# marco-conciatori-public/weed_instance_segmentation

Hardware: AMD Instinct MI355X
Metric: images/sec at 1024x1024 bs=8 per GPU (Mask2Former R50, 100 queries, fp32 forward-only) (higher is better)
Workload: dtype f32

## Files before the change

include/wm2f.h:

```cpp
#ifndef WM2F_H
#define WM2F_H

#include <stdint.h>

#ifdef __cplusplus
extern "C" {
#endif

#define WM2F_VERSION 100

#define WM2F_F32 0
#define WM2F_BF16 1
#define WM2F_I32 2
#define WM2F_U8 3
#define WM2F_U16 4
#define WM2F_I64 5

#define WM2F_OK 0
#define WM2F_EINVAL (-1)
#define WM2F_EUNSUPPORTED (-2)
#define WM2F_ELAUNCH (-3)

#define WM2F_MAX_LEVELS 8

// ... 181 lines not shown
                             int N, int Hi, int Wi, int stride, int relu, int config, int pieces, void* stream);
int wm2f_conv1x1_split_gn_fwd_p(const void* x, const void* w_split, const void* bias, void* out, void* stats_out, int G_out,
                                const void* norm_stats, const void* norm_gamma, const void* norm_beta, int norm_G, float norm_eps,
                                int norm_relu, int B, int K, int N, int Hi, int Wi, int stride, int config, int pieces,
                                void* stream);
int wm2f_conv1x1_split_dual_fwd_p(const void* x1, const void* ws1, const void* x2, const void* ws2, const void* bias, void* out,
                                  int B, int K1, int K2, int N, int Ho, int Wo, int H2, int W2, int stride2, int config,
                                  int pieces, void* stream);
int wm2f_conv3x3_split_fwd_p(const void* x, const void* w_split, const void* bias, void* out, int B, int Cin, int N, int Hi,
                             int Wi, int stride, int relu, int config, int pieces, void* stream);
int wm2f_conv3x3_split_stats_fwd_p(const void* x, const void* w_split, void* out, void* stats_out, int G_out, int B, int Cin,
                                   int N, int Hi, int Wi, int stride, int config, int pieces, void* stream);
int wm2f_stem7x7_pool_fwd_p(const void* x, const void* w_split, const void* bias, void* out, int B, int Cin, int N, int Hi,
                            int Wi, int grid, int pieces, void* stream);

int wm2f_swin_linear_split_fwd_p(const void* x, const void* w_split, const void* bias, const void* residual, void* out0,
                                 void* out1, void* out2, int64_t M, int K, int N, int epilogue, int n_out, int config,
                                 int pieces, void* stream);
int wm2f_swin_linear_split_config(int64_t M, int N, int pieces, int n_cu);
int wm2f_swin_linear_split_configs(void);

int64_t wm2f_token_wgrad_workspace(int64_t M, int N, int K);
int wm2f_token_wgrad_bf16(const void* dy, const void* x, void* dw, void* db, void* workspace, int64_t M, int N, int K,
                          void* stream);
int wm2f_token_wgrad_f32(const void* dy, const void* x, void* dw, void* db, void* workspace, int64_t M, int N, int K,
                         void* stream);
int wm2f_tokens_to_nchw(const void* tokens, void* out, int B, int S, int C, int start, int HW, void* stream);
int wm2f_group_norm_tokens(const void* x, const void* bias, const void* gamma, const void* beta, void* tokens,
                           void* stats_ws, int B, int C, int G, int HW, int S, int start, float eps, void* stream);
int wm2f_resize_bilinear(const void* x, void* y, int NC, int H, int W, int Ho, int Wo, void* stream);
// ... 261 lines not shown
```

weed_instance_segmentation_amd/_lib.py:

```python
from __future__ import annotations

import ctypes
import os
from ctypes import POINTER, c_char_p, c_float, c_int, c_int32, c_int64, c_void_p

HERE = os.path.dirname(os.path.abspath(__file__))
LIB_PATH = os.path.join(HERE, "libwm2f.so")
PROF_LIB_PATH = os.path.join(HERE, "libwm2f_prof.so")
if os.environ.get("WM2F_PROF_LIB"):
    PROF_LIB_PATH = os.environ["WM2F_PROF_LIB"]

WM2F_F32 = 0
WM2F_BF16 = 1
WM2F_I32 = 2
WM2F_U8 = 3
WM2F_U16 = 4
WM2F_I64 = 5
WM2F_CCL_VALUE, WM2F_CCL_BINARY, WM2F_CCL_RGB = 0, 1, 2
WM2F_CCL_MAX_COLORS = 16
WM2F_POLY_MAX_SIDE = 16384
WM2F_POLY_MAX_COORD = 1 << 24
WM2F_RLE_MAX_IDS = 1024
WM2F_AUG_MAX_VIRTUAL = 65536
WM2F_TILE_MAX_SIDE, WM2F_TILE_MAX_IDS, WM2F_TILE_MAX_TILES, WM2F_TILE_MAX_PAIRS = 16384, 256, 1024, 16384
# ... 85 lines not shown
    "wm2f_conv3x3_split_config": (c_int, [_I, _I, _I, _I]),
    "wm2f_conv3x3_split_fwd": (c_int, [_P, _P, _P, _P, _I, _I, _I, _I, _I, _I, _I, _I, _P]),
    "wm2f_conv1x1_split_gn_fwd": (c_int, [_P, _P, _P, _P, _P, _I, _P, _P, _P, _I, c_float, _I, _I, _I, _I, _I, _I, _I, _I, _P]),
    "wm2f_conv3x3_split_stats_fwd": (c_int, [_P, _P, _P, _P, _I, _I, _I, _I, _I, _I, _I, _I, _P]),
    "wm2f_group_norm_act_apply": (c_int, [_P, _P, _P, _P, _P, _P, _I, _I, _I, _I, _I, _I, _I, c_float, _I, _P]),
    "wm2f_group_norm_tokens_apply": (c_int, [_P, _P, _P, _P, _P, _P, _I, _I, _I, _I, _I, _I, c_float, _P]),
    "wm2f_stem7x7_pool_fwd":(c_int, [_P, _P, _P, _P, _I, _I, _I, _I, _I, _I, _P]),
    "wm2f_token_linear_split_fwd_p": (c_int, [_P, _P, _P, _P, _P, _P, _P, _P, _P, c_int64, _I, _I, _I, c_int64, c_float, _I, _I, _P]),
    "wm2f_token_ffn_split_fwd_p": (c_int, [_P, _P, _P, _P, _P, _P, _P, _P, _P, _P, _P, c_int64, _I, _I, _I, c_int64, c_float, _I, _P]),
    "wm2f_conv1x1_split_fwd_p": (c_int, [_P, _P, _P, _P, _P, _I, _I, _I, _I, _I, _I, _I, _I, _I, _P]),
    "wm2f_conv1x1_split_gn_fwd_p": (c_int, [_P, _P, _P, _P, _P, _I, _P, _P, _P, _I, c_float, _I, _I, _I, _I, _I, _I, _I, _I, _I, _P]),
    "wm2f_conv1x1_split_dual_fwd_p": (c_int, [_P, _P, _P, _P, _P, _P, _I, _I, _I, _I, _I, _I, _I, _I, _I, _I, _I, _P]),
    "wm2f_conv3x3_split_fwd_p": (c_int, [_P, _P, _P, _P, _I, _I, _I, _I, _I, _I, _I, _I, _I, _P]),
    "wm2f_conv3x3_split_stats_fwd_p": (c_int, [_P, _P, _P, _P, _I, _I, _I, _I, _I, _I, _I, _I, _I, _P]),
    "wm2f_stem7x7_pool_fwd_p": (c_int, [_P, _P, _P, _P, _I, _I, _I, _I, _I, _I, _I, _P]),
    "wm2f_swin_linear_split_fwd_p": (c_int, [_P, _P, _P, _P, _P, _P, _P, c_int64, _I, _I, _I, _I, _I, _I, _P]),
    "wm2f_swin_linear_split_config": (c_int, [c_int64, _I, _I, _I]),
    "wm2f_swin_linear_split_configs": (c_int, []),
    "wm2f_token_wgrad_workspace": (c_int64, [c_int64, _I, _I]),
    "wm2f_token_wgrad_bf16": (c_int, [_P, _P, _P, _P, _P, c_int64, _I, _I, _P]),
    "wm2f_token_wgrad_f32": (c_int, [_P, _P, _P, _P, _P, c_int64, _I, _I, _P]),
    "wm2f_tokens_to_nchw": (c_int, [_P, _P, _I, _I, _I, _I, _I, _P]),
    "wm2f_group_norm_tokens": (c_int, [_P, _P, _P, _P, _P, _P, _I, _I, _I, _I, _I, _I, c_float, _P]),
    "wm2f_resize_bilinear": (c_int, [_P, _P, _I, _I, _I, _I, _I, _P]),
    "wm2f_resize_pyramid": (c_int, [_P, _P, _P, _P, _I, _I, _I, _P]),
    "wm2f_bias_relu_maxpool": (c_int, [_P, _P, _P, _I, _I, _I, _I, _P]),
    "wm2f_group_norm_act": (c_int, [_P, _P, _P, _P, _P, _P, _I, _I, _I, _I, _I, _I, _I, c_float, _I, _P]),
    "wm2f_point_sample_fwd": (c_int, [_P, _I, _P, _P, _P, _I, _I, _I, _I, _P]),
    "wm2f_point_sample_bwd": (c_int, [_P, _P, _P, _P, _I, _I, _I, _I, _P]),
    "wm2f_labelmap_pair_counts": (c_int, [_P, _I, _P, _I, _P, _P, _P, _I, c_int64, _I, _I, _P]),
# ... 126 lines not shown
```

weed_instance_segmentation_amd/csrc/conv3x3_split.hip:

```cpp
#include "common.h"
#include "group_norm.h"

namespace wm2f {
namespace {

using f32x4 = __attribute__((ext_vector_type(4))) float;
using f32x8 = __attribute__((ext_vector_type(8))) float;
using bf16x8 = __attribute__((ext_vector_type(8))) __bf16;
typedef __attribute__((address_space(3))) void* lds_ptr_t;

constexpr int kWaves = 8;
constexpr int kThreads = kWaves * 64;
constexpr int kCT = 2;
constexpr int kKStep = 32;
constexpr int kFrag = 1024;
constexpr unsigned kOob = 0x80000000u;
constexpr float kBf16Max = 3.38953139e38f;

enum : int { kRaw = 0, kBias = 1, kBiasRelu = 2 };

__device__ __forceinline__ f32x8 widen(const bf16x8 v) {
  using u32x4 = __attribute__((ext_vector_type(4))) unsigned;
  const u32x4 w = __builtin_bit_cast(u32x4, v);
  f32x8 r;
// ... 21 lines not shown
    if constexpr (P >= 3) {
      const f32x8 r2 = r1 - widen(m);
      l = __builtin_convertvector(r2, bf16x8);
    }
  }
}

struct C3Args {
  const float *x, *bias;
  const void* ws;
  float* out;
  int Cin, N;
  int Hi, Wi, Wo, P, stride;
  double* stats;
  int G, cpg;
};

__device__ __forceinline__ void c3_barrier() {
  asm volatile("s_waitcnt vmcnt(0)" ::: "memory");
  __builtin_amdgcn_s_barrier();
  asm volatile("" ::: "memory");
}

template <int NRT, int WN, int EPI, bool STATS = false, int P = 3>
__global__ __launch_bounds__(kThreads) void conv3x3_split_kernel(C3Args a) {
  static_assert(P >= 1 && P <= 3, "one, two or three pieces");
  extern __shared__ __attribute__((aligned(16))) unsigned char smem[];
  constexpr int kRowTiles = WN * NRT;
  constexpr int kPanelBytes = kRowTiles * P * kFrag;
  constexpr int kPieces = kRowTiles * P;
  constexpr int kPT = (kWaves / WN) * kCT * 16;
  const int tid = threadIdx.x, lane = tid & 63, wave = __builtin_amdgcn_readfirstlane(tid >> 6);
  const int wn = wave % WN, wp = wave / WN;
  const int g = lane >> 4, j = lane & 15;
  const int nb = blockIdx.x, b = blockIdx.z;
  const int n_wg = nb * kRowTiles * 16;
  const int p_w = blockIdx.y * kPT + wp * kCT * 16;
  const int n_cb = a.Cin / kKStep;
  const int n_ks = 9 * n_cb;
  const int HWi = a.Hi * a.Wi;

// ... 20 lines not shown
    tap_ok[c] = m;
  }
  const unsigned ch_bytes = (unsigned)HWi * 4;

  f32x8 xr[kCT];
  auto issue = [&](int it) {
    const int cb = it / 9, tap = it - 9 * cb;
    const int dy = tap / 3, dx = tap - 3 * dy;
    unsigned char* dst = smem + (it & 1) * kPanelBytes;
    const int src = ((tap * n_cb + cb) * (a.N / 16) + n_wg / 16) * 3 * kFrag;
    for (int f = wave; f < kPieces; f += kWaves) {
      const int fs = P == 3 ? f : (f / P) * 3 + f % P;
      __builtin_amdgcn_raw_ptr_buffer_load_lds(w_rs, (lds_ptr_t)(dst + f * kFrag), 16, lane * 16, src + fs * kFrag, 0, 0);
    }
    const int kb = (cb * kKStep * HWi + dy * a.Wi + dx) * 4;
#pragma unroll
    for (int c = 0; c < kCT; ++c) {
      const unsigned o = (tap_ok[c] >> tap) & 1u ? (unsigned)(xo[c] + kb) : kOob;
#pragma unroll
      for (int i = 0; i < 8; ++i)
        xr[c][i] = __builtin_bit_cast(float, __builtin_amdgcn_raw_buffer_load_b32(x_rs, o, i * ch_bytes, 0));
    }
  };

  issue(0);
  c3_barrier();

  f32x4 acc[NRT][kCT];
#pragma unroll
  for (int rt = 0; rt < NRT; ++rt)
#pragma unroll
    for (int c = 0; c < kCT; ++c) acc[rt][c] = (f32x4){0.f, 0.f, 0.f, 0.f};

  for (int it = 0; it < n_ks; ++it) {
    bf16x8 bh[kCT], bm[kCT], bl[kCT];
#pragma unroll
    for (int c = 0; c < kCT; ++c) split3<P>(xr[c], bh[c], bm[c], bl[c]);
    if (it + 1 < n_ks) issue(it + 1);

    const unsigned char* panel = smem + (it & 1) * kPanelBytes + wn * NRT * P * kFrag;
    auto read_a = [&](bf16x8 (&dst)[3], int rt) {
#pragma unroll
      for (int p = 0; p < P; ++p) dst[p] = *reinterpret_cast<const bf16x8*>(panel + (rt * P + p) * kFrag + lane * 16);
    };
    auto six = [&](f32x4 acc_in, const bf16x8 (&av)[3], int cc) {
      f32x4 c = {0.f, 0.f, 0.f, 0.f};
      if constexpr (P == 3) {
        c = __builtin_amdgcn_mfma_f32_16x16x32_bf16(av[1], bm[cc], c, 0, 0, 0);
        c = __builtin_amdgcn_mfma_f32_16x16x32_bf16(av[2], bh[cc], c, 0, 0, 0);
        c = __builtin_amdgcn_mfma_f32_16x16x32_bf16(av[0], bl[cc], c, 0, 0, 0);
      }
      if constexpr (P >= 2) {
// ... 36 lines not shown
      for (int e = 0; e < 4; ++e) {
        float v = acc[rt][c][e];
        if (EPI != kRaw) v += bv[e];
        if (EPI == kBiasRelu) v = v < 0.f ? 0.f : v;
        __builtin_amdgcn_raw_buffer_store_b32(__builtin_bit_cast(unsigned, v), o_rs, ro, e * rs, 0);
        if (STATS && p < a.P) {
          gs[rt] += v;
          gss[rt] = fmaf(v, v, gss[rt]);
        }
      }
    }
  }
  if (STATS) gn_tile_stats<NRT, WN, kWaves>(gs, gss, smem, a.stats, b * a.G, n_wg, a.cpg, tid);
}

struct Cfg {
  int nrt, wn;
};
constexpr Cfg kCfg[] = {{16, 1}, {8, 2}, {4, 4}, {8, 1}, {4, 1}};
constexpr int kNumCfg = sizeof(kCfg) / sizeof(kCfg[0]);

template <int NRT, int WN, int P>
void (*pick_epi(int epi, bool stats))(C3Args) {
  if (stats) return conv3x3_split_kernel<NRT, WN, kRaw, true, P>;
  switch (epi) {
    case kRaw: return conv3x3_split_kernel<NRT, WN, kRaw, false, P>;
    case kBias: return conv3x3_split_kernel<NRT, WN, kBias, false, P>;
    default: return conv3x3_split_kernel<NRT, WN, kBiasRelu, false, P>;
  }
}

template <int P>
void (*pick_cfg(int ci, int epi, bool stats))(C3Args) {
  switch (ci) {
    case 0: return pick_epi<16, 1, P>(epi, stats);
    case 1: return pick_epi<8, 2, P>(epi, stats);
    case 2: return pick_epi<4, 4, P>(epi, stats);
    case 3: return pick_epi<8, 1, P>(epi, stats);
    default: return pick_epi<4, 1, P>(epi, stats);
  }
}

void (*pick_kernel(int ci, int epi, bool stats, int pieces))(C3Args) {
  return pieces == 3 ? pick_cfg<3>(ci, epi, stats) : (pieces == 2 ? pick_cfg<2>(ci, epi, stats) : pick_cfg<1>(ci, epi, stats));
}

int choose_cfg(int N, int P, int B, int n_cu) {
  int best = -1;
  int64_t best_cost = 0;
  for (int i = 0; i < kNumCfg; ++i) {
    const int nt = kCfg[i].wn * kCfg[i].nrt * 16, pt = (kWaves / kCfg[i].wn) * kCT * 16;
    if (N % nt) continue;
    const int64_t wgs = (int64_t)(N / nt) * ceil_div(P, pt) * B;
    const int64_t cost = ceil_div64(wgs, n_cu) * (kCfg[i].nrt + 4);
    if (best < 0 || cost < best_cost || (cost == best_cost && kCfg[i].wn < kCfg[best].wn)) best = i, best_cost = cost;
  }
  return best;
}

int cu_count(int* n_cu) {
  int dev = 0;
  if (hipGetDevice(&dev) != hipSuccess) return -1;
  static int cached[64] = {0};
  if (dev < 0 || dev >= 64) return -1;
  if (cached[dev] == 0) {
    hipDeviceProp_t prop;
    if (hipGetDeviceProperties(&prop, dev) != hipSuccess) return -1;
    cached[dev] = prop.multiProcessorCount;
  }
  *n_cu = cached[dev];
  return 0;
}

}
}

using namespace wm2f;

extern "C" int wm2f_conv3x3_split_config(int N, int P, int B, int n_cu) {
  if (N <= 0 || P <= 0 || B <= 0 || n_cu <= 0) return -1;
  return choose_cfg(N, P, B, n_cu);
}

static int conv3x3_launch(const char* who, const void* x, const void* w_split, const void* bias, void* out, void* stats_out,
                          int G_out, int B, int Cin, int N, int Hi, int Wi, int stride, int relu, int config, int pieces,
                          void* stream) {
  WM2F_REQUIRE(pieces >= 1 && pieces <= 3, "%s: pieces = %d (1, 2 and 3 are built)", who, pieces);
  WM2F_REQUIRE(x && w_split && out, "%s: null pointer", who);
  WM2F_REQUIRE(B > 0 && Cin > 0 && N > 0 && Hi > 0 && Wi > 0, "%s: non-positive size", who);
  WM2F_REQUIRE(Cin % kKStep == 0 && N % 64 == 0, "%s: Cin = %d must be a multiple of %d and N = %d of 64", who, Cin, kKStep, N);
  WM2F_REQUIRE(stride == 1 || stride == 2, "%s: stride %d (1 and 2 are built)", who, stride);
  const int Ho = (Hi - 1) / stride + 1, Wo = (Wi - 1) / stride + 1;
  const int64_t P = (int64_t)Ho * Wo;
  WM2F_REQUIRE((int64_t)Cin * Hi * Wi * 4 < (1ll << 31) && (int64_t)N * P * 4 < (1ll << 31),
               "%s: one image of x / out must stay below 2 GiB (32-bit buffer offsets)", who);
  WM2F_REQUIRE((int64_t)N * 9 * Cin * 6 < (1ll << 31), "%s: the split weight must stay below 2 GiB", who);
  WM2F_REQUIRE(!relu || bias, "%s: the ReLU epilogue carries a bias", who);
  if (stats_out) {
    WM2F_REQUIRE(!bias && !relu, "%s: the statistics epilogue is built for the raw output", who);
    WM2F_REQUIRE(G_out > 0 && N % G_out == 0 && gn_epilogue_cpg(N / G_out),
                 "%s: N = %d in %d groups: the epilogue reduces groups of 4, 8 or 16 channels", who, N, G_out);
  }
  int n_cu = 0;
  if (cu_count(&n_cu) != 0) {
    set_error("%s: cannot query the device", who);
    return WM2F_ELAUNCH;
  }
  WM2F_REQUIRE(config >= -1 && config < kNumCfg, "%s: configuration %d out of range", who, config);
  const int ci = config >= 0 ? config : choose_cfg(N, (int)P, B, n_cu);
  WM2F_REQUIRE(ci >= 0 && N % (kCfg[ci].wn * kCfg[ci].nrt * 16) == 0, "%s: no configuration %d for N = %d", who, ci, N);
  const int epi = relu ? kBiasRelu : (bias ? kBias : kRaw);
  const int nt = kCfg[ci].wn * kCfg[ci].nrt * 16, pt = (kWaves / kCfg[ci].wn) * kCT * 16;
  C3Args a;
  a.x = (const float*)x;
  a.ws = w_split;
  a.bias = (const float*)bias;
  a.out = (float*)out;
  a.Cin = Cin;
  a.N = N;
  a.Hi = Hi;
  a.Wi = Wi;
  a.Wo = Wo;
  a.P = (int)P;
  a.stride = stride;
  a.stats = (double*)stats_out;
  a.G = stats_out ? G_out : 1;
  a.cpg = stats_out ? N / G_out : 4;
  const size_t lds = (size_t)2 * (nt / 16) * pieces * kFrag;
  void (*kfn)(C3Args) = pick_kernel(ci, epi, stats_out != nullptr, pieces);
  hipError_t e = hipFuncSetAttribute((const void*)kfn, hipFuncAttributeMaxDynamicSharedMemorySize, (int)lds);
  if (e != hipSuccess) {
    set_error("%s: cannot raise dynamic LDS to %zu: %s", who, lds, hipGetErrorString(e));
    return WM2F_ELAUNCH;
  }
  if (stats_out) {
    e = hipMemsetAsync(stats_out, 0, sizeof(double) * 2 * B * G_out, (hipStream_t)stream);
    WM2F_REQUIRE(e == hipSuccess, "%s: memset failed: %s", who, hipGetErrorString(e));
  }
  hipLaunchKernelGGL(kfn, dim3(N / nt, ceil_div((int)P, pt), B), dim3(kThreads), lds, (hipStream_t)stream, a);
  WM2F_CHECK_LAUNCH(who);
  return WM2F_OK;
}

extern "C" int wm2f_conv3x3_split_fwd(const void* x, const void* w_split, const void* bias, void* out, int B, int Cin, int N,
                                      int Hi, int Wi, int stride, int relu, int config, void* stream) {
  return conv3x3_launch("wm2f_conv3x3_split_fwd", x, w_split, bias, out, nullptr, 0, B, Cin, N, Hi, Wi, stride, relu, config,
                        3, stream);
}

extern "C" int wm2f_conv3x3_split_fwd_p(const void* x, const void* w_split, const void* bias, void* out, int B, int Cin, int N,
                                        int Hi, int Wi, int stride, int relu, int config, int pieces, void* stream) {
  return conv3x3_launch("wm2f_conv3x3_split_fwd_p", x, w_split, bias, out, nullptr, 0, B, Cin, N, Hi, Wi, stride, relu, config,
                        pieces, stream);
}

extern "C" int wm2f_conv3x3_split_stats_fwd(const void* x, const void* w_split, void* out, void* stats_out, int G_out, int B,
                                            int Cin, int N, int Hi, int Wi, int stride, int config, void* stream) {
  const char* who = "wm2f_conv3x3_split_stats_fwd";
  WM2F_REQUIRE(stats_out, "%s: null pointer", who);
  return conv3x3_launch(who, x, w_split, nullptr, out, stats_out, G_out, B, Cin, N, Hi, Wi, stride, 0, config, 3, stream);
}

extern "C" int wm2f_conv3x3_split_stats_fwd_p(const void* x, const void* w_split, void* out, void* stats_out, int G_out, int B,
                                              int Cin, int N, int Hi, int Wi, int stride, int config, int pieces, void* stream) {
  const char* who = "wm2f_conv3x3_split_stats_fwd_p";
  WM2F_REQUIRE(stats_out, "%s: null pointer", who);
  return conv3x3_launch(who, x, w_split, nullptr, out, stats_out, G_out, B, Cin, N, Hi, Wi, stride, 0, config, pieces, stream);
}
```

weed_instance_segmentation_amd/ops/__init__.py:

```python
from __future__ import annotations

import os as _os

K1_BWD_DETERMINISTIC: bool | None = None

CONV1X1_SPLIT = True

CONV3X3_SPLIT = True

CONV_GN_FUSED = True

SHORTCUT_FOLD = True

TOKEN_FFN_FUSED = True

SWIN_LINEAR_SPLIT: bool | tuple = ("highest", "high", "medium")

SPLIT_PRECISION: str | None = _os.environ.get("WM2F_SPLIT_PRECISION") or "highest"

from .._lib import check
from ._core import KernelTimer, _p, _stream, set_kernel_timer
from .ccl import label_components, resize_nearest_tables
from .clean import labelmap_clean
from .copy_paste import copy_paste
from .fused import (add_broadcast, bias_act_, bias_relu_maxpool, group_norm_act_, group_norm_act_from_stats_, group_norm_tokens_,
                    group_norm_tokens_from_stats_, resize_bilinear, resize_pyramid, tokens_to_nchw)
from .gemm import (conv1x1, conv1x1_applies, conv1x1_dual, conv1x1_dual_applies, conv1x1_gn, conv3x3, conv3x3_applies, conv3x3_stats, conv_group_stats_applies,
                   ROWS_FFN, ROWS_NATURAL, ffn_row_order, linear_tokens, split_weight, split_weight_3x3,
                   split_weight_cached, split_weight_rows, split_weight_rows_cached, split_weight_stem, stem_conv_pool,
                   stem_conv_pool_applies, stem_weight_columns, stem_weight_matrix, swin_linear, swin_linear_applies,
                   token_ffn, token_ffn_applies,
                   token_linear, token_linear_applies, token_wgrad, token_wgrad_applies)
from .k1 import (k1_bwd_deterministic, k1_lane_order, k1_lane_rows, k1_lanes_applies, k1_rows_applies, ms_deform_attn,
                 ms_deform_attn_bwd, ms_deform_attn_fused, ms_deform_attn_fused_lanes, ms_deform_attn_fused_packed,
                 ms_deform_attn_rows, ms_deform_attn_variant)
from .k2 import masked_xattn, masked_xattn_bf16_applies
from .k3 import (attn_mask_build, mask_einsum, mask_einsum_attn_mask, mask_einsum_bf16, mask_einsum_bf16_bwd,
                 mask_einsum_bf16_bwd_applies, mask_einsum_bwd, mask_einsum_bwd_applies, nchw_to_pixel_major_bf16)
from .labelmaps import (cell_grid_shape, coco_match, coco_match_min, labelmap_aim_points, labelmap_boundary,
                        labelmap_cell_counts, labelmap_distance, labelmap_hull, labelmap_instance_stats, labelmap_nearest,
                        labelmap_pair_counts, labelmap_shape_stats, labelmap_to_masks, mask_pair_counts, panoptic_match,
                        semantic_confusion_)
# ... 18 lines not shown
```

weed_instance_segmentation_amd/ops/gemm.py:

```python
from __future__ import annotations

import torch

from .. import ops as _flags
from .._lib import Wm2fError, load
from ..derived import derived
from ._core import _launch, _p, _req
from .fused import bias_act_, bias_relu_maxpool


_LEVEL_PIECES = {None: 3, "highest": 3, "high": 2, "medium": 1}


def _split_pieces():
    level = _flags.SPLIT_PRECISION
    if not (level is None or isinstance(level, str)) or level not in _LEVEL_PIECES:
        raise ValueError(f"ops.SPLIT_PRECISION = {level!r}: 'highest', 'high', 'medium' or None")
    pieces = _LEVEL_PIECES[level]
    return pieces, ("" if pieces == 3 else f"_p{pieces}")


def token_linear_applies(x: torch.Tensor, weight: torch.Tensor) -> bool:
    N, K = weight.shape
    M = x.numel() // max(K, 1)
# ... 324 lines not shown
    if norm is not None:
        nstats, nG, ngamma, nbeta, neps, nrelu = norm
        nstats, ngamma, nbeta = _req(nstats, "norm stats", torch.float64), _req(ngamma, "gamma"), _req(nbeta, "beta")
        if nstats.numel() != 2 * B * int(nG) or ngamma.shape != (K,) or nbeta.shape != (K,):
            raise ValueError("conv1x1_gn: norm = (stats (B, G, 2) fp64, G, gamma (K), beta (K), eps, relu)")
    else:
        stats = torch.empty(B, int(stats_groups), 2, device=x.device, dtype=torch.float64)
    out = torch.empty(B, N, Ho, Wo, device=x.device, dtype=torch.float32)
    pieces, lvl = _split_pieces()
    _launch("wm2f_conv1x1_split_gn_fwd_p", x, _p(x), _p(w_split), _p(bias), _p(out), _p(stats), int(stats_groups), _p(nstats),
            _p(ngamma), _p(nbeta), int(nG), float(neps), 1 if nrelu else 0, B, K, N, H, W, int(stride), int(config), pieces,
            tag=f"conv1x1_K{K}_N{N}_P{Ho * Wo}{lvl}")
    return out if norm is not None else (out, stats)


def conv3x3_stats(x: torch.Tensor, weight: torch.Tensor, groups: int, stride: int = 1, w_split: torch.Tensor | None = None,
                  config: int = -1):
    if not conv3x3_applies(x, weight, stride):
        raise ValueError("conv3x3_stats: shapes outside conv3x3_applies take conv3x3 and the separate GroupNorm passes")
    x = _req(x, "x")
    N, Cin = int(weight.shape[0]), int(weight.shape[1])
    B, _, H, W = x.shape
    Ho, Wo = (H - 1) // stride + 1, (W - 1) // stride + 1
    if w_split is None:
        w_split = split_weight_3x3(_req(weight, "weight"))
    else:
        _check_split(w_split, N * 9 * Cin * 6, x, "conv3x3_stats: w_split is not split_weight_3x3(weight)")
    out = torch.empty(B, N, Ho, Wo, device=x.device, dtype=torch.float32)
    stats = torch.empty(B, int(groups), 2, device=x.device, dtype=torch.float64)
    pieces, lvl = _split_pieces()
    _launch("wm2f_conv3x3_split_stats_fwd_p", x, _p(x), _p(w_split), _p(out), _p(stats), int(groups), B, Cin, N, H, W,
            int(stride), int(config), pieces, tag=f"conv3x3_C{Cin}_N{N}_P{Ho * Wo}{lvl}")
    return out, stats


def conv3x3_applies(x: torch.Tensor, weight: torch.Tensor, stride: int = 1) -> bool:
    if x.dim() != 4 or weight.dim() != 4 or tuple(weight.shape[2:]) != (3, 3):
        return False
    N, C = int(weight.shape[0]), int(weight.shape[1])
    _, K, H, W = x.shape
    Ho, Wo = (H - 1) // stride + 1, (W - 1) // stride + 1
    return (x.is_cuda and x.dtype == torch.float32 and weight.dtype == torch.float32 and C == K and K % 32 == 0
            and N % 64 == 0 and stride in (1, 2) and K * H * W * 4 < (1 << 31) and N * Ho * Wo * 4 < (1 << 31)
            and N * 9 * K * 6 < (1 << 31))


def conv3x3(x: torch.Tensor, weight: torch.Tensor, bias: torch.Tensor | None = None, relu: bool = False, stride: int = 1,
            split: bool = True, w_split: torch.Tensor | None = None, config: int = -1) -> torch.Tensor:
    if relu and bias is None:
        raise ValueError("conv3x3: the ReLU epilogue carries a bias")
    if not split or not conv3x3_applies(x, weight, stride):
        y = torch.nn.functional.conv2d(x, weight, None, stride, 1)
        if bias is None:
            return y
        if (y.shape[-1] * y.shape[-2]) % 4 == 0:
            return bias_act_(y, bias, None, relu)
        y = y + bias[None, :, None, None]
        return torch.relu(y) if relu else y
    x = _req(x, "x")
    N, Cin = int(weight.shape[0]), int(weight.shape[1])
    B, _, H, W = x.shape
    Ho, Wo = (H - 1) // stride + 1, (W - 1) // stride + 1
    if bias is not None:
        bias = _req(bias, "bias")
        if bias.shape != (N,):
            raise ValueError(f"conv3x3: bias {tuple(bias.shape)} for {N} channels")
    if w_split is None:
        w_split = split_weight_3x3(_req(weight, "weight"))
    else:
        _check_split(w_split, N * 9 * Cin * 6, x, "conv3x3: w_split is not split_weight_3x3(weight)")
    out = torch.empty(B, N, Ho, Wo, device=x.device, dtype=torch.float32)
    pieces, lvl = _split_pieces()
    _launch("wm2f_conv3x3_split_fwd_p", x, _p(x), _p(w_split), _p(bias), _p(out), B, Cin, N, H, W, int(stride),
            1 if relu else 0, int(config), pieces, tag=f"conv3x3_C{Cin}_N{N}_P{Ho * Wo}{lvl}")
    return out


STEM_K = 160


def stem_weight_columns(cin: int) -> torch.Tensor:
    if cin not in (1, 2, 3):
        raise ValueError(f"stem_weight_columns: Cin = {cin} (1, 2 and 3 are built)")
    cols = torch.full((STEM_K,), -1, dtype=torch.long)
    rows = 7 * cin
    for G in range(min(rows, STEM_K // 8)):
        cols[8 * G:8 * G + 7] = torch.arange(7 * G, 7 * G + 7)
    if rows > STEM_K // 8:
        cols[7:8 * 7:8] = torch.arange(7 * 20, 7 * 21)
# ... 105 lines not shown
```

Baseline: 304.9.

## Add staged conv3x3 kernel that splits a halo tile once into LDS

Adds a staged 3x3 convolution path. Each workgroup loads an 8x32 spatial tile plus its halo, splits it into bf16 pieces once, and stores them in LDS, so all nine taps read from there instead of reloading and resplitting the input per tap. A host-side routing rule turns the path on for stride-1, single-wave-column configs that fit the LDS limit and divide the spatial size evenly, and it is enabled by default through a new flag. It also adds profiling-only ablation variants of the direct kernel. The cost is higher LDS use and possibly lower occupancy, plus more code and template variants.

```diff
diff --git a/include/wm2f.h b/include/wm2f.h
--- a/include/wm2f.h
+++ b/include/wm2f.h
@@ -219,6 +219,12 @@
 int wm2f_stem7x7_pool_fwd_p(const void* x, const void* w_split, const void* bias, void* out, int B, int Cin, int N, int Hi,
                             int Wi, int grid, int pieces, void* stream);
 
+int wm2f_conv3x3_split_fwd_r(const void* x, const void* w_split, const void* bias, void* out, int B, int Cin, int N, int Hi,
+                             int Wi, int stride, int relu, int config, int pieces, int route, void* stream);
+int wm2f_conv3x3_split_stats_fwd_r(const void* x, const void* w_split, void* out, void* stats_out, int G_out, int B, int Cin,
+                                   int N, int Hi, int Wi, int stride, int config, int pieces, int route, void* stream);
+int wm2f_conv3x3_split_route(int N, int Hi, int Wi, int stride, int B, int n_cu, int pieces, int* entry);
+
 int wm2f_swin_linear_split_fwd_p(const void* x, const void* w_split, const void* bias, const void* residual, void* out0,
                                  void* out1, void* out2, int64_t M, int K, int N, int epilogue, int n_out, int config,
                                  int pieces, void* stream);
diff --git a/weed_instance_segmentation_amd/_lib.py b/weed_instance_segmentation_amd/_lib.py
--- a/weed_instance_segmentation_amd/_lib.py
+++ b/weed_instance_segmentation_amd/_lib.py
@@ -123,6 +123,9 @@
     "wm2f_conv3x3_split_fwd_p": (c_int, [_P, _P, _P, _P, _I, _I, _I, _I, _I, _I, _I, _I, _I, _P]),
     "wm2f_conv3x3_split_stats_fwd_p": (c_int, [_P, _P, _P, _P, _I, _I, _I, _I, _I, _I, _I, _I, _I, _P]),
     "wm2f_stem7x7_pool_fwd_p": (c_int, [_P, _P, _P, _P, _I, _I, _I, _I, _I, _I, _I, _P]),
+    "wm2f_conv3x3_split_fwd_r": (c_int, [_P, _P, _P, _P, _I, _I, _I, _I, _I, _I, _I, _I, _I, _I, _P]),
+    "wm2f_conv3x3_split_stats_fwd_r": (c_int, [_P, _P, _P, _P, _I, _I, _I, _I, _I, _I, _I, _I, _I, _I, _P]),
+    "wm2f_conv3x3_split_route": (c_int, [_I, _I, _I, _I, _I, _I, _I, _P]),
     "wm2f_swin_linear_split_fwd_p": (c_int, [_P, _P, _P, _P, _P, _P, _P, c_int64, _I, _I, _I, _I, _I, _I, _P]),
     "wm2f_swin_linear_split_config": (c_int, [c_int64, _I, _I, _I]),
     "wm2f_swin_linear_split_configs": (c_int, []),
diff --git a/weed_instance_segmentation_amd/csrc/conv3x3_split.hip b/weed_instance_segmentation_amd/csrc/conv3x3_split.hip
--- a/weed_instance_segmentation_amd/csrc/conv3x3_split.hip
+++ b/weed_instance_segmentation_amd/csrc/conv3x3_split.hip
@@ -59,6 +59,7 @@
   int Hi, Wi, Wo, P, stride;
   double* stats;
   int G, cpg;
+  int tiles_w;
 };
 
 __device__ __forceinline__ void c3_barrier() {
@@ -67,9 +68,11 @@
   asm volatile("" ::: "memory");
 }
 
-template <int NRT, int WN, int EPI, bool STATS = false, int P = 3>
+enum : int { kAblSplit = 1, kAblLoads = 2 };
+template <int NRT, int WN, int EPI, bool STATS = false, int P = 3, int ABL = 0>
 __global__ __launch_bounds__(kThreads) void conv3x3_split_kernel(C3Args a) {
   static_assert(P >= 1 && P <= 3, "one, two or three pieces");
+  static_assert(ABL == 0 || P == 3, "the ablations are built for three pieces");
   extern __shared__ __attribute__((aligned(16))) unsigned char smem[];
   constexpr int kRowTiles = WN * NRT;
   constexpr int kPanelBytes = kRowTiles * P * kFrag;
@@ -120,6 +123,7 @@
       __builtin_amdgcn_raw_ptr_buffer_load_lds(w_rs, (lds_ptr_t)(dst + f * kFrag), 16, lane * 16, src + fs * kFrag, 0, 0);
     }
     const int kb = (cb * kKStep * HWi + dy * a.Wi + dx) * 4;
+    if (ABL == kAblLoads && tap != 0) return;
 #pragma unroll
     for (int c = 0; c < kCT; ++c) {
       const unsigned o = (tap_ok[c] >> tap) & 1u ? (unsigned)(xo[c] + kb) : kOob;
@@ -138,10 +142,23 @@
 #pragma unroll
     for (int c = 0; c < kCT; ++c) acc[rt][c] = (f32x4){0.f, 0.f, 0.f, 0.f};
 
+  bf16x8 kh[kCT], km[kCT], kl[kCT];
   for (int it = 0; it < n_ks; ++it) {
     bf16x8 bh[kCT], bm[kCT], bl[kCT];
-#pragma unroll
-    for (int c = 0; c < kCT; ++c) split3<P>(xr[c], bh[c], bm[c], bl[c]);
+    if (ABL == 0 || it % 9 == 0) {
+#pragma unroll
+      for (int c = 0; c < kCT; ++c) split3<P>(xr[c], bh[c], bm[c], bl[c]);
+      if constexpr (ABL != 0) {
+#pragma unroll
+        for (int c = 0; c < kCT; ++c) kh[c] = bh[c], km[c] = bm[c], kl[c] = bl[c];
+      }
+    } else {
+#pragma unroll
+      for (int c = 0; c < kCT; ++c) {
+        bh[c] = kh[c], bm[c] = km[c], bl[c] = kl[c];
+        if constexpr (ABL == kAblSplit) asm volatile("" ::"v"(xr[c]));
+      }
+    }
     if (it + 1 < n_ks) issue(it + 1);
 
     const unsigned char* panel = smem + (it & 1) * kPanelBytes + wn * NRT * P * kFrag;
@@ -208,6 +225,178 @@
   if (STATS) gn_tile_stats<NRT, WN, kWaves>(gs, gss, smem, a.stats, b * a.G, n_wg, a.cpg, tid);
 }
 
+constexpr int kTH = 8, kTW = 32;
+constexpr int kHW = kTW + 2, kHalo = (kTH + 2) * kHW;
+constexpr int kStageItems = 4 * kHalo;
+constexpr int kStageRounds = (kStageItems + kThreads - 1) / kThreads;
+constexpr int kStagePiece = kStageItems * 16;
+static_assert(kTH == kWaves && kTW == kCT * 16, "a wave owns one row of the tile");
+
+template <int NRT, int EPI, bool STATS = false, int P = 3>
+__global__ __launch_bounds__(kThreads) void conv3x3_staged_kernel(C3Args a) {
+  static_assert(P >= 1 && P <= 3, "one, two or three pieces");
+  extern __shared__ __attribute__((aligned(16))) unsigned char smem[];
+  constexpr int kPanelBytes = NRT * P * kFrag;
+  constexpr int kPieces = NRT * P;
+  unsigned char* const tile = smem + 2 * kPanelBytes;
+  const int tid = threadIdx.x, lane = tid & 63, wave = __builtin_amdgcn_readfirstlane(tid >> 6);
+  const int g = lane >> 4, j = lane & 15;
+  const int nb = blockIdx.x, b = blockIdx.z;
+  const int n_wg = nb * NRT * 16;
+  const int ty = blockIdx.y / a.tiles_w, tx = blockIdx.y - ty * a.tiles_w;
+  const int h0 = ty * kTH, w0 = tx * kTW;
+  const int n_cb = a.Cin / kKStep;
+  const int HWi = a.Hi * a.Wi;
+
+  const __amdgpu_buffer_rsrc_t w_rs = __builtin_amdgcn_make_buffer_rsrc((void*)a.ws, 0, a.N * 9 * a.Cin * 6, 0x00020000);
+  const __amdgpu_buffer_rsrc_t x_rs =
+      __builtin_amdgcn_make_buffer_rsrc((void*)(a.x + (int64_t)b * a.Cin * HWi), 0, a.Cin * HWi * 4, 0x00020000);
+
+  unsigned so[kStageRounds];
+#pragma unroll
+  for (int r = 0; r < kStageRounds; ++r) {
+    const int s = r * kThreads + tid;
+    const int sg = s / kHalo, hp = s - sg * kHalo;
+    const int hy = hp / kHW, hx = hp - hy * kHW;
+    const int hi = h0 - 1 + hy, wi = w0 - 1 + hx;
+    const bool ok = s < kStageItems && (unsigned)hi < (unsigned)a.Hi && (unsigned)wi < (unsigned)a.Wi;
+    so[r] = ok ? (unsigned)(((8 * sg) * HWi + hi * a.Wi + wi) * 4) : kOob;
+  }
+  const unsigned ch_bytes = (unsigned)HWi * 4;
+
+  f32x8 xs[kStageRounds];
+  auto stage_load = [&](int r, int cb) {
+    const unsigned o = so[r] != kOob ? so[r] + (unsigned)(cb * kKStep) * ch_bytes : kOob;
+#pragma unroll
+    for (int i = 0; i < 8; ++i)
+      xs[r][i] = __builtin_bit_cast(float, __builtin_amdgcn_raw_buffer_load_b32(x_rs, o, i * ch_bytes, 0));
+  };
+  auto stage_write = [&]() {
+#pragma unroll
+    for (int r = 0; r < kStageRounds; ++r) {
+      bf16x8 pc[3];
+      split3<P>(xs[r], pc[0], pc[1], pc[2]);
+      const int s = r * kThreads + tid;
+      if (s < kStageItems) {
+#pragma unroll
+        for (int p = 0; p < P; ++p) *reinterpret_cast<bf16x8*>(tile + p * kStagePiece + s * 16) = pc[p];
+      }
+    }
+  };
+  auto issue_a = [&](int it, int cb, int tap) {
+    unsigned char* dst = smem + (it & 1) * kPanelBytes;
+    const int src = ((tap * n_cb + cb) * (a.N / 16) + n_wg / 16) * 3 * kFrag;
+    for (int f = wave; f < kPieces; f += kWaves) {
+      const int fs = P == 3 ? f : (f / P) * 3 + f % P;
+      __builtin_amdgcn_raw_ptr_buffer_load_lds(w_rs, (lds_ptr_t)(dst + f * kFrag), 16, lane * 16, src + fs * kFrag, 0, 0);
+    }
+  };
+
+  issue_a(0, 0, 0);
+#pragma unroll
+  for (int r = 0; r < kStageRounds; ++r) stage_load(r, 0);
+  c3_barrier();
+  stage_write();
+  __syncthreads();
+
+  f32x4 acc[NRT][kCT];
+#pragma unroll
+  for (int rt = 0; rt < NRT; ++rt)
+#pragma unroll
+    for (int c = 0; c < kCT; ++c) acc[rt][c] = (f32x4){0.f, 0.f, 0.f, 0.f};
+
+  const unsigned char* const bsrc = tile + (g * kHalo + wave * kHW + j) * 16;
+  int it = 0;
+#pragma unroll 1
+  for (int cb = 0; cb < n_cb; ++cb) {
+#pragma unroll 1
+    for (int tap = 0; tap < 9; ++tap, ++it) {
+      const int dy = tap / 3, dx = tap - 3 * dy;
+      bf16x8 bf[kCT][3];
+#pragma unroll
+      for (int c = 0; c < kCT; ++c)
+#pragma unroll
+        for (int p = 0; p < P; ++p)
+          bf[c][p] = *reinterpret_cast<const bf16x8*>(bsrc + (dy * kHW + dx) * 16 + c * 256 + p * kStagePiece);
+      const bool last = tap == 8 && cb + 1 == n_cb;
+      if (!last) issue_a(it + 1, tap == 8 ? cb + 1 : cb, tap == 8 ? 0 : tap + 1);
+      if (cb + 1 < n_cb) {
+#pragma unroll
+        for (int r = 0; r < kStageRounds; ++r)
+          if (tap == 3 * r) stage_load(r, cb + 1);
+      }
+
+      const unsigned char* panel = smem + (it & 1) * kPanelBytes;
+      auto read_a = [&](bf16x8 (&dst)[3], int rt) {
+#pragma unroll
+        for (int p = 0; p < P; ++p) dst[p] = *reinterpret_cast<const bf16x8*>(panel + (rt * P + p) * kFrag + lane * 16);
+      };
+      auto six = [&](f32x4 acc_in, const bf16x8 (&av)[3], int cc) {
+        f32x4 c = {0.f, 0.f, 0.f, 0.f};
+        if constexpr (P == 3) {
+          c = __builtin_amdgcn_mfma_f32_16x16x32_bf16(av[1], bf[cc][1], c, 0, 0, 0);
+          c = __builtin_amdgcn_mfma_f32_16x16x32_bf16(av[2], bf[cc][0], c, 0, 0, 0);
+          c = __builtin_amdgcn_mfma_f32_16x16x32_bf16(av[0], bf[cc][2], c, 0, 0, 0);
+        }
+        if constexpr (P >= 2) {
+          c = __builtin_amdgcn_mfma_f32_16x16x32_bf16(av[1], bf[cc][0], c, 0, 0, 0);
+          c = __builtin_amdgcn_mfma_f32_16x16x32_bf16(av[0], bf[cc][1], c, 0, 0, 0);
+        }
+        return acc_in + __builtin_amdgcn_mfma_f32_16x16x32_bf16(av[0], bf[cc][0], c, 0, 0, 0);
+      };
+      bf16x8 av[2][3];
+      read_a(av[0], 0);
+#pragma unroll
+      for (int rt = 0; rt < NRT; ++rt) {
+        if (rt + 1 < NRT) read_a(av[(rt + 1) & 1], rt + 1);
+        __builtin_amdgcn_sched_barrier(0);
+        acc[rt][0] = six(acc[rt][0], av[rt & 1], 0);
+        acc[rt][1] = six(acc[rt][1], av[rt & 1], 1);
+        __builtin_amdgcn_sched_barrier(0);
+      }
+      c3_barrier();
+    }
+    if (cb + 1 < n_cb) {
+      stage_write();
+      __syncthreads();
+    }
+  }
+
+  const int64_t img = (int64_t)b * a.N * a.P;
+  const __amdgpu_buffer_rsrc_t o_rs = __builtin_amdgcn_make_buffer_rsrc((void*)(a.out + img), 0, a.N * a.P * 4, 0x00020000);
+  const int n0 = n_wg + 4 * g;
+  const int ho = h0 + wave;
+  float gs[NRT], gss[NRT];
+#pragma unroll
+  for (int rt = 0; rt < NRT; ++rt) {
+    gs[rt] = gss[rt] = 0.f;
+    float bv[4] = {0.f, 0.f, 0.f, 0.f};
+    if (EPI != kRaw) {
+#pragma unroll
+      for (int e = 0; e < 4; ++e) bv[e] = a.bias[n0 + rt * 16 + e];
+    }
+#pragma unroll
+    for (int c = 0; c < kCT; ++c) {
+      const int wo = w0 + c * 16 + j;
+      const bool live = ho < a.Hi && wo < a.Wi;
+      const unsigned ro = live ? (unsigned)(((n0 + rt * 16) * a.P + ho * a.Wi + wo) * 4) : kOob;
+      const unsigned rs = (unsigned)a.P * 4;
+#pragma unroll
+      for (int e = 0; e < 4; ++e) {
+        float v = acc[rt][c][e];
+        if (EPI != kRaw) v += bv[e];
+        if (EPI == kBiasRelu) v = v < 0.f ? 0.f : v;
+        __builtin_amdgcn_raw_buffer_store_b32(__builtin_bit_cast(unsigned, v), o_rs, ro, e * rs, 0);
+        if (STATS && live) {
+          gs[rt] += v;
+          gss[rt] = fmaf(v, v, gss[rt]);
+        }
+      }
+    }
+  }
+  if (STATS) gn_tile_stats<NRT, 1, kWaves>(gs, gss, smem, a.stats, b * a.G, n_wg, a.cpg, tid);
+}
+
 struct Cfg {
   int nrt, wn;
 };
@@ -238,6 +427,58 @@
 void (*pick_kernel(int ci, int epi, bool stats, int pieces))(C3Args) {
   return pieces == 3 ? pick_cfg<3>(ci, epi, stats) : (pieces == 2 ? pick_cfg<2>(ci, epi, stats) : pick_cfg<1>(ci, epi, stats));
 }
+
+template <int NRT, int P>
+void (*pick_staged_epi(int epi, bool stats))(C3Args) {
+  if (stats) return conv3x3_staged_kernel<NRT, kRaw, true, P>;
+  switch (epi) {
+    case kRaw: return conv3x3_staged_kernel<NRT, kRaw, false, P>;
+    case kBias: return conv3x3_staged_kernel<NRT, kBias, false, P>;
+    default: return conv3x3_staged_kernel<NRT, kBiasRelu, false, P>;
+  }
+}
+
+template <int P>
+void (*pick_staged_cfg(int ci, int epi, bool stats))(C3Args) {
+  switch (kCfg[ci].nrt) {
+    case 16: return pick_staged_epi<16, P>(epi, stats);
+    case 8: return pick_staged_epi<8, P>(epi, stats);
+    default: return pick_staged_epi<4, P>(epi, stats);
+  }
+}
+
+void (*pick_staged(int ci, int epi, bool stats, int pieces))(C3Args) {
+  return pieces == 3 ? pick_staged_cfg<3>(ci, epi, stats)
+                     : (pieces == 2 ? pick_staged_cfg<2>(ci, epi, stats) : pick_staged_cfg<1>(ci, epi, stats));
+}
+
+#ifdef WM2F_PROFILING
+template <int NRT, int WN>
+void (*pick_abl_epi(int epi, int abl))(C3Args) {
+  if (abl == kAblSplit) {
+    switch (epi) {
+      case kRaw: return conv3x3_split_kernel<NRT, WN, kRaw, false, 3, kAblSplit>;
+      case kBias: return conv3x3_split_kernel<NRT, WN, kBias, false, 3, kAblSplit>;
+      default: return conv3x3_split_kernel<NRT, WN, kBiasRelu, false, 3, kAblSplit>;
+    }
+  }
+  switch (epi) {
+    case kRaw: return conv3x3_split_kernel<NRT, WN, kRaw, false, 3, kAblLoads>;
+    case kBias: return conv3x3_split_kernel<NRT, WN, kBias, false, 3, kAblLoads>;
+    default: return conv3x3_split_kernel<NRT, WN, kBiasRelu, false, 3, kAblLoads>;
+  }
+}
+
+void (*pick_abl(int ci, int epi, int abl))(C3Args) {
+  switch (ci) {
+    case 0: return pick_abl_epi<16, 1>(epi, abl);
+    case 1: return pick_abl_epi<8, 2>(epi, abl);
+    case 2: return pick_abl_epi<4, 4>(epi, abl);
+    case 3: return pick_abl_epi<8, 1>(epi, abl);
+    default: return pick_abl_epi<4, 1>(epi, abl);
+  }
+}
+#endif
 
 int choose_cfg(int N, int P, int B, int n_cu) {
   int best = -1;
@@ -252,6 +493,22 @@
   return best;
 }
 
+constexpr int kLdsLimit = 163840;
+
+int staged_lds(int nrt, int pieces) { return pieces * (2 * nrt * kFrag + kStagePiece); }
+
+int64_t staged_tiles(int Hi, int Wi) { return (int64_t)ceil_div(Hi, kTH) * ceil_div(Wi, kTW); }
+
+bool staged_applies(int ci, int Hi, int Wi, int stride, int pieces, int lds_limit) {
+  return stride == 1 && kCfg[ci].wn == 1 && staged_lds(kCfg[ci].nrt, pieces) <= lds_limit && staged_tiles(Hi, Wi) <= 65535;
+}
+
+bool staged_pays(int ci, int N, int Hi, int Wi, int B, int n_cu) {
+  if (Hi % kTH || Wi % kTW) return false;
+  const int64_t wgs = (int64_t)(N / (kCfg[ci].nrt * 16)) * B * staged_tiles(Hi, Wi);
+  return !(kCfg[ci].nrt == 4 && wgs > n_cu);
+}
+
 int cu_count(int* n_cu) {
   int dev = 0;
   if (hipGetDevice(&dev) != hipSuccess) return -1;
@@ -266,6 +523,20 @@
   return 0;
 }
 
+int lds_max(int* bytes) {
+  int dev = 0;
+  if (hipGetDevice(&dev) != hipSuccess) return -1;
+  static int cached[64] = {0};
+  if (dev < 0 || dev >= 64) return -1;
+  if (cached[dev] == 0) {
+    int v = 0;
+    if (hipDeviceGetAttribute(&v, hipDeviceAttributeMaxSharedMemoryPerBlock, dev) != hipSuccess || v <= 0) return -1;
+    cached[dev] = v;
+  }
+  *bytes = cached[dev];
+  return 0;
+}
+
 }
 }
 
@@ -276,9 +547,20 @@
   return choose_cfg(N, P, B, n_cu);
 }
 
+extern "C" int wm2f_conv3x3_split_route(int N, int Hi, int Wi, int stride, int B, int n_cu, int pieces, int* entry) {
+  if (N <= 0 || N % 64 || Hi <= 0 || Wi <= 0 || (stride != 1 && stride != 2) || B <= 0 || n_cu <= 0 || pieces < 1 || pieces > 3)
+    return -1;
+  const int64_t P = (int64_t)((Hi - 1) / stride + 1) * ((Wi - 1) / stride + 1);
+  if (P >= (1ll << 31)) return -1;
+  const int ci = choose_cfg(N, (int)P, B, n_cu);
+  if (ci < 0) return -1;
+  if (entry) *entry = ci;
+  return staged_applies(ci, Hi, Wi, stride, pieces, kLdsLimit) && staged_pays(ci, N, Hi, Wi, B, n_cu) ? 1 : 0;
+}
+
 static int conv3x3_launch(const char* who, const void* x, const void* w_split, const void* bias, void* out, void* stats_out,
                           int G_out, int B, int Cin, int N, int Hi, int Wi, int stride, int relu, int config, int pieces,
-                          void* stream) {
+                          int route, void* stream) {
   WM2F_REQUIRE(pieces >= 1 && pieces <= 3, "%s: pieces = %d (1, 2 and 3 are built)", who, pieces);
   WM2F_REQUIRE(x && w_split && out, "%s: null pointer", who);
   WM2F_REQUIRE(B > 0 && Cin > 0 && N > 0 && Hi > 0 && Wi > 0, "%s: non-positive size", who);
@@ -303,6 +585,17 @@
   WM2F_REQUIRE(config >= -1 && config < kNumCfg, "%s: configuration %d out of range", who, config);
   const int ci = config >= 0 ? config : choose_cfg(N, (int)P, B, n_cu);
   WM2F_REQUIRE(ci >= 0 && N % (kCfg[ci].wn * kCfg[ci].nrt * 16) == 0, "%s: no configuration %d for N = %d", who, ci, N);
+  WM2F_REQUIRE(route >= -1 && route <= 1, "%s: route %d (-1 auto, 0 direct, 1 staged)", who, route);
+  int lds_limit = kLdsLimit;
+  if (route != 0 && staged_applies(ci, Hi, Wi, stride, pieces, kLdsLimit) && lds_max(&lds_limit) != 0) {
+    set_error("%s: cannot query the device", who);
+    return WM2F_ELAUNCH;
+  }
+  const bool applies = staged_applies(ci, Hi, Wi, stride, pieces, lds_limit < kLdsLimit ? lds_limit : kLdsLimit);
+  WM2F_REQUIRE(route != 1 || applies,
+               "%s: the staged route is built for stride 1 on a WN = 1 entry within %d B of LDS (stride %d, entry %d, %d B)", who,
+               lds_limit, stride, ci, staged_lds(kCfg[ci].nrt, pieces));
+  const bool staged = route == 1 || (route < 0 && applies && staged_pays(ci, N, Hi, Wi, B, n_cu));
   const int epi = relu ? kBiasRelu : (bias ? kBias : kRaw);
   const int nt = kCfg[ci].wn * kCfg[ci].nrt * 16, pt = (kWaves / kCfg[ci].wn) * kCT * 16;
   C3Args a;
@@ -320,8 +613,18 @@
   a.stats = (double*)stats_out;
   a.G = stats_out ? G_out : 1;
   a.cpg = stats_out ? N / G_out : 4;
-  const size_t lds = (size_t)2 * (nt / 16) * pieces * kFrag;
-  void (*kfn)(C3Args) = pick_kernel(ci, epi, stats_out != nullptr, pieces);
+  a.tiles_w = ceil_div(Wi, kTW);
+  const size_t lds = staged ? (size_t)staged_lds(kCfg[ci].nrt, pieces) : (size_t)2 * (nt / 16) * pieces * kFrag;
+  void (*kfn)(C3Args) = staged ? pick_staged(ci, epi, stats_out != nullptr, pieces) : pick_kernel(ci, epi, stats_out != nullptr, pieces);
+#ifdef WM2F_PROFILING
+  if (!staged) {
+    const char* ea = getenv("WM2F_C3_ABL");
+    const int abl = ea ? atoi(ea) : 0;
+    WM2F_REQUIRE(abl == 0 || abl == kAblSplit || abl == kAblLoads, "%s: WM2F_C3_ABL = %d is not built (1 and 2 are)", who, abl);
+    WM2F_REQUIRE(abl == 0 || (pieces == 3 && !stats_out), "%s: WM2F_C3_ABL is built for three pieces without statistics", who);
+    if (abl) kfn = pick_abl(ci, epi, abl);
+  }
+#endif
   hipError_t e = hipFuncSetAttribute((const void*)kfn, hipFuncAttributeMaxDynamicSharedMemorySize, (int)lds);
   if (e != hipSuccess) {
     set_error("%s: cannot raise dynamic LDS to %zu: %s", who, lds, hipGetErrorString(e));
@@ -331,7 +634,8 @@
     e = hipMemsetAsync(stats_out, 0, sizeof(double) * 2 * B * G_out, (hipStream_t)stream);
     WM2F_REQUIRE(e == hipSuccess, "%s: memset failed: %s", who, hipGetErrorString(e));
   }
-  hipLaunchKernelGGL(kfn, dim3(N / nt, ceil_div((int)P, pt), B), dim3(kThreads), lds, (hipStream_t)stream, a);
+  const int grid_y = staged ? (int)staged_tiles(Hi, Wi) : ceil_div((int)P, pt);
+  hipLaunchKernelGGL(kfn, dim3(N / nt, grid_y, B), dim3(kThreads), lds, (hipStream_t)stream, a);
   WM2F_CHECK_LAUNCH(who);
   return WM2F_OK;
 }
@@ -339,25 +643,39 @@
 extern "C" int wm2f_conv3x3_split_fwd(const void* x, const void* w_split, const void* bias, void* out, int B, int Cin, int N,
                                       int Hi, int Wi, int stride, int relu, int config, void* stream) {
   return conv3x3_launch("wm2f_conv3x3_split_fwd", x, w_split, bias, out, nullptr, 0, B, Cin, N, Hi, Wi, stride, relu, config,
-                        3, stream);
+                        3, -1, stream);
 }
 
 extern "C" int wm2f_conv3x3_split_fwd_p(const void* x, const void* w_split, const void* bias, void* out, int B, int Cin, int N,
                                         int Hi, int Wi, int stride, int relu, int config, int pieces, void* stream) {
   return conv3x3_launch("wm2f_conv3x3_split_fwd_p", x, w_split, bias, out, nullptr, 0, B, Cin, N, Hi, Wi, stride, relu, config,
-                        pieces, stream);
+                        pieces, -1, stream);
 }
 
 extern "C" int wm2f_conv3x3_split_stats_fwd(const void* x, const void* w_split, void* out, void* stats_out, int G_out, int B,
                                             int Cin, int N, int Hi, int Wi, int stride, int config, void* stream) {
   const char* who = "wm2f_conv3x3_split_stats_fwd";
   WM2F_REQUIRE(stats_out, "%s: null pointer", who);
-  return conv3x3_launch(who, x, w_split, nullptr, out, stats_out, G_out, B, Cin, N, Hi, Wi, stride, 0, config, 3, stream);
+  return conv3x3_launch(who, x, w_split, nullptr, out, stats_out, G_out, B, Cin, N, Hi, Wi, stride, 0, config, 3, -1, stream);
 }
 
 extern "C" int wm2f_conv3x3_split_stats_fwd_p(const void* x, const void* w_split, void* out, void* stats_out, int G_out, int B,
                                               int Cin, int N, int Hi, int Wi, int stride, int config, int pieces, void* stream) {
   const char* who = "wm2f_conv3x3_split_stats_fwd_p";
   WM2F_REQUIRE(stats_out, "%s: null pointer", who);
-  return conv3x3_launch(who, x, w_split, nullptr, out, stats_out, G_out, B, Cin, N, Hi, Wi, stride, 0, config, pieces, stream);
-}
+  return conv3x3_launch(who, x, w_split, nullptr, out, stats_out, G_out, B, Cin, N, Hi, Wi, stride, 0, config, pieces, -1, stream);
+}
+
+extern "C" int wm2f_conv3x3_split_fwd_r(const void* x, const void* w_split, const void* bias, void* out, int B, int Cin, int N,
+                                        int Hi, int Wi, int stride, int relu, int config, int pieces, int route, void* stream) {
+  return conv3x3_launch("wm2f_conv3x3_split_fwd_r", x, w_split, bias, out, nullptr, 0, B, Cin, N, Hi, Wi, stride, relu, config,
+                        pieces, route, stream);
+}
+
+extern "C" int wm2f_conv3x3_split_stats_fwd_r(const void* x, const void* w_split, void* out, void* stats_out, int G_out, int B,
+                                              int Cin, int N, int Hi, int Wi, int stride, int config, int pieces, int route,
+                                              void* stream) {
+  const char* who = "wm2f_conv3x3_split_stats_fwd_r";
+  WM2F_REQUIRE(stats_out, "%s: null pointer", who);
+  return conv3x3_launch(who, x, w_split, nullptr, out, stats_out, G_out, B, Cin, N, Hi, Wi, stride, 0, config, pieces, route, stream);
+}
diff --git a/weed_instance_segmentation_amd/ops/__init__.py b/weed_instance_segmentation_amd/ops/__init__.py
--- a/weed_instance_segmentation_amd/ops/__init__.py
+++ b/weed_instance_segmentation_amd/ops/__init__.py
@@ -7,6 +7,8 @@
 CONV1X1_SPLIT = True
 
 CONV3X3_SPLIT = True
+
+CONV3X3_STAGED = True
 
 CONV_GN_FUSED = True
 
@@ -25,7 +27,7 @@
 from .copy_paste import copy_paste
 from .fused import (add_broadcast, bias_act_, bias_relu_maxpool, group_norm_act_, group_norm_act_from_stats_, group_norm_tokens_,
                     group_norm_tokens_from_stats_, resize_bilinear, resize_pyramid, tokens_to_nchw)
-from .gemm import (conv1x1, conv1x1_applies, conv1x1_dual, conv1x1_dual_applies, conv1x1_gn, conv3x3, conv3x3_applies, conv3x3_stats, conv_group_stats_applies,
+from .gemm import (conv1x1, conv1x1_applies, conv1x1_dual, conv1x1_dual_applies, conv1x1_gn, conv3x3, conv3x3_applies, conv3x3_route, conv3x3_stats, conv3x3_stats_route, conv_group_stats_applies,
                    ROWS_FFN, ROWS_NATURAL, ffn_row_order, linear_tokens, split_weight, split_weight_3x3,
                    split_weight_cached, split_weight_rows, split_weight_rows_cached, split_weight_stem, stem_conv_pool,
                    stem_conv_pool_applies, stem_weight_columns, stem_weight_matrix, swin_linear, swin_linear_applies,
diff --git a/weed_instance_segmentation_amd/ops/gemm.py b/weed_instance_segmentation_amd/ops/gemm.py
--- a/weed_instance_segmentation_amd/ops/gemm.py
+++ b/weed_instance_segmentation_amd/ops/gemm.py
@@ -362,8 +362,21 @@
     return out if norm is not None else (out, stats)
 
 
+def _conv3x3_route(route: int | None) -> int:
+    if route is None:
+        return -1 if _flags.CONV3X3_STAGED else 0
+    if route not in (-1, 0, 1):
+        raise ValueError(f"conv3x3: route = {route!r}: None, -1 (the host's rule), 0 (direct) or 1 (staged)")
+    return int(route)
+
+
 def conv3x3_stats(x: torch.Tensor, weight: torch.Tensor, groups: int, stride: int = 1, w_split: torch.Tensor | None = None,
                   config: int = -1):
+    return conv3x3_stats_route(x, weight, groups, None, stride, w_split, config)
+
+
+def conv3x3_stats_route(x: torch.Tensor, weight: torch.Tensor, groups: int, route: int | None, stride: int = 1,
+                        w_split: torch.Tensor | None = None, config: int = -1):
     if not conv3x3_applies(x, weight, stride):
         raise ValueError("conv3x3_stats: shapes outside conv3x3_applies take conv3x3 and the separate GroupNorm passes")
     x = _req(x, "x")
@@ -377,8 +390,8 @@
     out = torch.empty(B, N, Ho, Wo, device=x.device, dtype=torch.float32)
     stats = torch.empty(B, int(groups), 2, device=x.device, dtype=torch.float64)
     pieces, lvl = _split_pieces()
-    _launch("wm2f_conv3x3_split_stats_fwd_p", x, _p(x), _p(w_split), _p(out), _p(stats), int(groups), B, Cin, N, H, W,
-            int(stride), int(config), pieces, tag=f"conv3x3_C{Cin}_N{N}_P{Ho * Wo}{lvl}")
+    _launch("wm2f_conv3x3_split_stats_fwd_r", x, _p(x), _p(w_split), _p(out), _p(stats), int(groups), B, Cin, N, H, W,
+            int(stride), int(config), pieces, _conv3x3_route(route), tag=f"conv3x3_C{Cin}_N{N}_P{Ho * Wo}{lvl}")
     return out, stats
 
 
@@ -395,6 +408,15 @@
 
 def conv3x3(x: torch.Tensor, weight: torch.Tensor, bias: torch.Tensor | None = None, relu: bool = False, stride: int = 1,
             split: bool = True, w_split: torch.Tensor | None = None, config: int = -1) -> torch.Tensor:
+    return _conv3x3(x, weight, bias, relu, stride, split, w_split, config, None)
+
+
+def conv3x3_route(x: torch.Tensor, weight: torch.Tensor, route: int | None, bias: torch.Tensor | None = None, relu: bool = False,
+                  stride: int = 1, w_split: torch.Tensor | None = None, config: int = -1) -> torch.Tensor:
+    return _conv3x3(x, weight, bias, relu, stride, True, w_split, config, route)
+
+
+def _conv3x3(x, weight, bias, relu, stride, split, w_split, config, route):
     if relu and bias is None:
         raise ValueError("conv3x3: the ReLU epilogue carries a bias")
     if not split or not conv3x3_applies(x, weight, stride):
@@ -419,8 +441,8 @@
         _check_split(w_split, N * 9 * Cin * 6, x, "conv3x3: w_split is not split_weight_3x3(weight)")
     out = torch.empty(B, N, Ho, Wo, device=x.device, dtype=torch.float32)
     pieces, lvl = _split_pieces()
-    _launch("wm2f_conv3x3_split_fwd_p", x, _p(x), _p(w_split), _p(bias), _p(out), B, Cin, N, H, W, int(stride),
-            1 if relu else 0, int(config), pieces, tag=f"conv3x3_C{Cin}_N{N}_P{Ho * Wo}{lvl}")
+    _launch("wm2f_conv3x3_split_fwd_r", x, _p(x), _p(w_split), _p(bias), _p(out), B, Cin, N, H, W, int(stride),
+            1 if relu else 0, int(config), pieces, _conv3x3_route(route), tag=f"conv3x3_C{Cin}_N{N}_P{Ho * Wo}{lvl}")
     return out
 
 
```

Result: faster. 311.0, median of 6 (+2.0%).
